# Zhengjun-Du/LC-CRF-SLAM

Measured on AMD Instinct MI355X. Metric: CRF mean-field iters/sec, higher is better.
Workload: dtype f32; 1 GPU; C2: 2000 keypoints, 5 iters, two 2-D kernels (TUM3.yaml), L=2; frames_in_flight_per_gpu=16384, handles=1, distinct_frames=64, n_points=2000, n_iters=5, n_labels=2, engine=fused

## Files before the change

### lc-crf-slam_amd/csrc/fused_lean.h

```cpp
#pragma once

#include "fused_loop.h"

#ifndef LCCRF_LEAN_SKIP
#define LCCRF_LEAN_SKIP 0
#endif
#define LEAN_SKIP(bit) ((LCCRF_LEAN_SKIP & (bit)) != 0)

namespace lccrf {
namespace fl {

constexpr int kLeanMaxRounds = 4;
__host__ __device__ constexpr int lean_rounds(int nt) { return nt >= 512 ? 3 : 4; }
__host__ __device__ constexpr int lean_max_v(int nt) { return 3 * (nt - 64); }

__host__ __device__ inline int lean_plane_floats(int NA, int V0)
{
    const int top = V0 < kChainTop ? V0 : kChainTop;
    return (NA * kD1 + 11 * top + 3 * (V0 - top) + 16 + 63) & ~63;
}

__host__ __device__ inline bool lean_chain_wanted(int NA, int V0, int row0, int nt)
{
    return row0 >= kChainMinRow && V0 <= chain_max_v(nt) && V0 <= 256 && lean_plane_floats(NA, V0) < 65535;
}

struct LeanTables {
    int val0, val1, nbr, row;
};
__host__ __device__ inline LeanTables lean_tables(size_t &o, int Vk, bool chain)
{
    auto take = [&](size_t bytes) { size_t r = o; o += (bytes + 15) & ~(size_t)15; return (int)r; };
    LeanTables t;
    t.val0 = take((size_t)(Vk + 1) * sizeof(float2));
    t.val1 = take((size_t)(Vk + 1) * sizeof(float2));
    t.nbr = chain ? take((size_t)kD1 * Vk * sizeof(unsigned)) : -1;
    t.row = take((size_t)(Vk + 2) * sizeof(unsigned short));
    return t;
}

__host__ __device__ inline bool layout_lean(int NA, int K, const int *V, int row0, FusedLayout *lay, int nt, size_t lds_limit)
{
    constexpr int D1 = kD1;
    if (NA < 1 || K < 1 || K > kMaxFusedK) return false;
    for (int k = 0; k < K; ++k)
        if (V[k] >= 65535 || V[k] > lean_max_v(nt)) return false;
    if (row0 >= kChainMinRow && !lean_chain_wanted(NA, V[0], row0, nt)) return false;
    const int chain0 = lean_chain_wanted(NA, V[0], row0, nt);
    {
        FusedLayout L{};
        size_t o = 0;
        auto take = [&](size_t bytes) { size_t r = o; o += (bytes + 15) & ~(size_t)15; return (int)r; };
        L.prod_all = 0;
        L.chain0 = chain0;
        L.zero = take(128);
        size_t shared_prod = 0;
        for (int k = 0; k < K; ++k) {
            const bool chain = k == 0 && chain0;
            L.Ecap[k] = chain ? lean_plane_floats(NA, V[k]) : ((NA * D1 + 63) & ~63);
            const LeanTables lt = lean_tables(o, V[k], chain);
            L.val[k][0] = lt.val0;
            L.val[k][1] = lt.val1;
            L.nbr[k] = lt.nbr;
            L.row[k] = lt.row;
            const size_t pb = (size_t)L.Ecap[k] * 2 * sizeof(float);
            shared_prod = pb > shared_prod ? pb : shared_prod;
        }
        if (o > 65535) return false;
        L.pstart = chain0 ? take((size_t)(V[0] + 2) * sizeof(unsigned short)) : 0;
        const int p = take(shared_prod < 1024 ? 1024 : shared_prod);
        for (int k = 0; k < K; ++k) L.prod[k] = p;
        L.total = (int)o;
        if (o <= lds_limit) {
            *lay = L;
            return true;
        }
    }
    return false;
}

#define LCCRF_ASM_SEL(off, vlo, vhi, S)                                                                             \
    "v_cmp_lt_i32_e32 vcc, " #off ", %[rem]\n\tv_cndmask_b32_e32 %[" #S "], 0, %[ad], vcc\n\t"                     \
    "ds_read_b128 v[" #vlo ":" #vhi "], %[" #S "] offset:" #off "\n\t"

__device__ __forceinline__ float chain_rows_sel(unsigned addr, int bytes, unsigned trips, unsigned &keep0, unsigned &keep1)
{
    float acc = 0.0f;
    if (trips == 0) return acc;
    unsigned sa, sb;
    asm volatile(
        LCCRF_ASM_SEL(0, 96, 99, sa) LCCRF_ASM_SEL(16, 100, 103, sb)
        LCCRF_ASM_SEL(32, 104, 107, sa) LCCRF_ASM_SEL(48, 108, 111, sb)
        LCCRF_ASM_SEL(64, 112, 115, sa) LCCRF_ASM_SEL(80, 116, 119, sb)
        "1:\n\t"
        LCCRF_ASM_SEL(96, 120, 123, sa) LCCRF_ASM_SEL(112, 124, 127, sb)
        "s_waitcnt lgkmcnt(6)\n\t"
        LCCRF_ASM_ADD8(v96, v97, v98, v99, v100, v101, v102, v103)
        "v_add_u32_e32 %[ad], 0x80, %[ad]\n\t"
        "v_subrev_u32_e32 %[rem], 0x80, %[rem]\n\t"
        LCCRF_ASM_SEL(0, 96, 99, sa) LCCRF_ASM_SEL(16, 100, 103, sb)
        "s_waitcnt lgkmcnt(6)\n\t"
        LCCRF_ASM_ADD8(v104, v105, v106, v107, v108, v109, v110, v111)
        LCCRF_ASM_SEL(32, 104, 107, sa) LCCRF_ASM_SEL(48, 108, 111, sb)
        "s_waitcnt lgkmcnt(6)\n\t"
        LCCRF_ASM_ADD8(v112, v113, v114, v115, v116, v117, v118, v119)
        LCCRF_ASM_SEL(64, 112, 115, sa) LCCRF_ASM_SEL(80, 116, 119, sb)
        "s_waitcnt lgkmcnt(6)\n\t"
        LCCRF_ASM_ADD8(v120, v121, v122, v123, v124, v125, v126, v127)
        "s_sub_u32 %[n], %[n], 1\n\t"
        "s_cmp_lg_u32 %[n], 0\n\t"
        "s_cbranch_scc1 1b\n\t"
        "s_waitcnt lgkmcnt(0)\n\t"
        : [acc] "+v"(acc), [ad] "+v"(addr), [rem] "+v"(bytes), [n] "+s"(trips), [sa] "=&v"(sa), [sb] "=&v"(sb), "+v"(keep0), "+v"(keep1)
        :
        : "scc", "vcc", "memory", LCCRF_CHAIN_RING_CLOBBERS);
    return acc;
}

__device__ __forceinline__ float chain_rows_keep(unsigned addr, unsigned end, unsigned trips, unsigned &keep0, unsigned &keep1)
{
    float acc = 0.0f;
    if (trips == 0) return acc;
    const unsigned e1 = end - 32u, e2 = end - 64u, e3 = end - 96u;
    unsigned sel;
    asm volatile(LCCRF_CHAIN_ROWS_ASM
                 : [acc] "+v"(acc), [ad] "+v"(addr), [n] "+s"(trips), [sel] "=&v"(sel), "+v"(keep0), "+v"(keep1)
                 : [e0] "v"(end), [e1] "v"(e1), [e2] "v"(e2), [e3] "v"(e3)
                 : "scc", "memory", LCCRF_CHAIN_RING_CLOBBERS);
    return acc;
}

__device__ __forceinline__ float2 lds_f2(unsigned addr)
{
#if defined(__HIP_DEVICE_COMPILE__)
    typedef float lean_f2 __attribute__((ext_vector_type(2)));
    const lean_f2 v = *reinterpret_cast<const __attribute__((address_space(3))) lean_f2 *>((unsigned long)addr);
    return make_float2(v.x, v.y);
#else
    (void)addr;
    return make_float2(0.f, 0.f);
#endif
}

__device__ __forceinline__ void lds_store_f(unsigned addr, float v)
{
#if defined(__HIP_DEVICE_COMPILE__)
    *reinterpret_cast<__attribute__((address_space(3))) float *>((unsigned long)addr) = v;
#else
    (void)addr; (void)v;
#endif
}
__device__ __forceinline__ void lds_store_f2(unsigned addr, float a, float b)
{
#if defined(__HIP_DEVICE_COMPILE__)
    typedef float lean_f2 __attribute__((ext_vector_type(2)));
    lean_f2 v;
    v.x = a;
    v.y = b;
    *reinterpret_cast<__attribute__((address_space(3))) lean_f2 *>((unsigned long)addr) = v;
#else
    (void)addr; (void)a; (void)b;
#endif
}

template <int PPT, int K, int CH>
__device__ __forceinline__ void point_products_lean(const FusedLayout &lay, const PointRegs<PPT, K> &pr, int s, int k)
{
    const unsigned a0 = (pr.ix[s][k][1] >> 16) << 2, a1 = (pr.ix[s][k][2] & 0xffffu) << 2, a2 = (pr.ix[s][k][2] >> 16) << 2;
    if (chain_k<CH>(lay, k)) {
        const unsigned pb = (unsigned)lay.Ecap[k] * 4u;
        lds_store_f(a0, pr.bary[s][k][0] * pr.q[s].x);
        lds_store_f(a0 + pb, pr.bary[s][k][0] * pr.q[s].y);
        lds_store_f(a1, pr.bary[s][k][1] * pr.q[s].x);
        lds_store_f(a1 + pb, pr.bary[s][k][1] * pr.q[s].y);
        lds_store_f(a2, pr.bary[s][k][2] * pr.q[s].x);
        lds_store_f(a2 + pb, pr.bary[s][k][2] * pr.q[s].y);
    } else {
        lds_store_f2(a0, pr.bary[s][k][0] * pr.q[s].x, pr.bary[s][k][0] * pr.q[s].y);
        lds_store_f2(a1, pr.bary[s][k][1] * pr.q[s].x, pr.bary[s][k][1] * pr.q[s].y);
        lds_store_f2(a2, pr.bary[s][k][2] * pr.q[s].x, pr.bary[s][k][2] * pr.q[s].y);
    }
}

template <int PPT, int K>
__device__ __forceinline__ float2 slice_point_lean(const PointRegs<PPT, K> &pr, int s, int k, float alpha)
{
    const float2 x0 = lds_f2(pr.ix[s][k][0] & 0xffffu), x1 = lds_f2(pr.ix[s][k][0] >> 16), x2 = lds_f2(pr.ix[s][k][1] & 0xffffu);
    const float w0 = pr.bary[s][k][0] * alpha, w1 = pr.bary[s][k][1] * alpha, w2 = pr.bary[s][k][2] * alpha;
    float t0 = w0 * x0.x, t1 = w0 * x0.y;
    t0 += w1 * x1.x; t1 += w1 * x1.y;
    t0 += w2 * x2.x; t1 += w2 * x2.y;
    return make_float2(t0, t1);
}

template <int NT>
__device__ __forceinline__ ChainLane chain_setup_lean(unsigned char *smem, const FusedLayout &lay, int V0, int tid)
{
    constexpr int k = 0;
    ChainLane cl{0u, 0u};
    int *hist = reinterpret_cast<int *>(smem + lay.prod[k]);
    if (tid < 128) hist[tid] = 0;
    __syncthreads();
    const unsigned short *row = reinterpret_cast<const unsigned short *>(smem + lay.row[k]);
    unsigned short *srt = reinterpret_cast<unsigned short *>(smem + lay.prod[k]) + 256;
    unsigned short *pstart = reinterpret_cast<unsigned short *>(smem + lay.pstart);
    int key = 0;
    if (tid < V0) {
        const int len = (int)row[tid + 1] - (int)row[tid];
        key = 63 - min((len + 3) >> 4, 63);
        atomicAdd(&hist[key], 1);
    }
    __syncthreads();
    if (tid < 64) {
        const int x = hist[tid];
        int incl = x;
#pragma unroll
        for (int o = 1; o < 64; o <<= 1) {
            const int y = __shfl_up(incl, o, 64);
            if (tid >= o) incl += y;
        }
        hist[64 + tid] = incl - x;
    }
    __syncthreads();
    if (tid < V0) srt[atomicAdd(&hist[64 + key], 1)] = (unsigned short)tid;
    __syncthreads();
    if (tid < 64) {
        int sz[4], sum = 0;
#pragma unroll
        for (int u = 0; u < 4; ++u) {
            const int r = tid * 4 + u;
            sz[u] = 0;
            if (r < V0) {
                const int v = srt[r];
                const int rl = (int)row[v + 1] - (int)row[v];
                sz[u] = ((rl + 3) & ~3) + (r < kChainTop ? 8 : 0);
            }
            sum += sz[u];
        }
        int incl = sum;
#pragma unroll
        for (int o = 1; o < 64; o <<= 1) {
            const int y = __shfl_up(incl, o, 64);
            if (tid >= o) incl += y;
        }
        int base = incl - sum;
#pragma unroll
        for (int u = 0; u < 4; ++u) {
            const int r = tid * 4 + u;
            if (r < V0) pstart[srt[r]] = (unsigned short)base;
            base += sz[u];
        }
    }
    __syncthreads();
    const int l = (tid >> 6) & 1, pr = tid >> 7, ln = tid & 63;
    const int r = pr == 0 ? (chain_top_rank(ln) >= 0 ? chain_top_rank(ln) : V0) : kChainTop + ((pr - 1) << 6) + ln;
    unsigned quads = 0, addr = 0;
    if (r < V0) {
        const int v = srt[r];
        const int rl = (int)row[v + 1] - (int)row[v], len4 = (rl + 3) & ~3;
        addr = (unsigned)(lay.prod[k] + 4 * (l * lay.Ecap[k] + (int)pstart[v]));
        quads = (unsigned)(len4 >> 2);
        cl.b = quads | ((unsigned)(len4 - rl) << 13) | ((unsigned)((v + 1) * 2 + l) << 16);
    }
    unsigned m = quads;
#pragma unroll
    for (int o = 32; o > 0; o >>= 1) m = max(m, (unsigned)__shfl_xor((int)m, o));
    cl.a = addr | (m << 18);
    __syncthreads();
    return cl;
}

__device__ __forceinline__ void chain_pads_lean(unsigned char *smem, const ChainLane &cl, int tid)
{
    if (cl.b >> 16) {
        float *e = reinterpret_cast<float *>(smem + (cl.a & 0x3ffffu)) + (cl.b & 0x1fffu) * 4u;
        const unsigned npad = (cl.b >> 13) & 3u;
        for (unsigned z = 1; z <= npad; ++z) e[-(int)z] = 0.0f;
        if ((tid >> 7) == 0) {
            reinterpret_cast<float4 *>(e)[0] = make_float4(0.f, 0.f, 0.f, 0.f);
            reinterpret_cast<float4 *>(e)[1] = make_float4(0.f, 0.f, 0.f, 0.f);
        }
    }
}

template <int PPT, int K, int CH, int NT>
__device__ __forceinline__ void place_products_lean(unsigned char *smem, const FusedLayout &lay, int N, int tid,
                                                    const unsigned (&pk)[PPT][K][kD1], PointRegs<PPT, K> &pr)
{
#pragma unroll
    for (int k = 0; k < K; ++k) {
        const unsigned short *row = reinterpret_cast<const unsigned short *>(smem + lay.row[k]);
        const unsigned short *pstart = reinterpret_cast<const unsigned short *>(smem + lay.pstart);
#pragma unroll
        for (int s = 0; s < PPT; ++s) {
            const unsigned vb = (unsigned)lay.val[k][kD1 & 1];
            pr.ix[s][k][0] = (vb + 8u * (pk[s][k][0] & 0xffffu)) | ((vb + 8u * (pk[s][k][1] & 0xffffu)) << 16);
            pr.ix[s][k][1] = vb + 8u * (pk[s][k][2] & 0xffffu);
            pr.ix[s][k][2] = 0;
            if (tid + s * NT < N) {
                unsigned sl[kD1];
#pragma unroll
                for (int j = 0; j < kD1; ++j) {
                    sl[j] = pk[s][k][j] >> 16;
                    if (chain_k<CH>(lay, k)) {
                        const int v = (int)(pk[s][k][j] & 0xffffu) - 1;
                        sl[j] = (unsigned)((int)pstart[v] + ((int)(pk[s][k][j] >> 16) - (int)row[v]));
                        sl[j] = ((unsigned)lay.prod[k] >> 2) + sl[j];
                    } else {
                        sl[j] = ((unsigned)lay.prod[k] >> 2) + 2u * sl[j];
                    }
                }
                pr.ix[s][k][1] |= sl[0] << 16;
                pr.ix[s][k][2] = sl[1] | (sl[2] << 16);
            }
        }
    }
}

typedef unsigned lean_u3 __attribute__((ext_vector_type(3)));
struct LeanSrc {
    __amdgpu_buffer_rsrc_t nbr[kMaxFusedK];
    __amdgpu_buffer_rsrc_t bary[kMaxFusedK];
    __amdgpu_buffer_rsrc_t norm[kMaxFusedK];
    __amdgpu_buffer_rsrc_t unary;
    int nbr_axis_bytes[kMaxFusedK];
    int off_nbr[kMaxFusedK], off_bary[kMaxFusedK], off_norm[kMaxFusedK], off_unary;
};
constexpr int kLeanRecPoints = 4 * kNTSmall;
constexpr int kLeanRecUnary = 0;
constexpr int kLeanRecBary = kLeanRecUnary + kLeanRecPoints * 8;
constexpr int kLeanRecNorm = kLeanRecBary + kMaxFusedK * kLeanRecPoints * kD1 * 4;
constexpr int kLeanRecNbr = kLeanRecNorm + kMaxFusedK * kLeanRecPoints * 4;
constexpr int kLeanRecNbrAxis = lean_max_v(kNTSmall) * 4;
constexpr int kLeanRecBytes = (kLeanRecNbr + kD1 * kLeanRecNbrAxis + 255) & ~255;
__device__ __forceinline__ __amdgpu_buffer_rsrc_t lean_rsrc(const void *p, size_t bytes)
{
    return __builtin_amdgcn_make_buffer_rsrc(const_cast<void *>(p), 0, (int)bytes, 0x00020000);
}

template <int PPT, int K>
__device__ __forceinline__ void opaque_ids(PointRegs<PPT, K> &pr)
{
#pragma unroll
    for (int s = 0; s < PPT; ++s) {
#pragma unroll
        for (int k = 0; k < K; ++k) asm volatile("" : "+v"(pr.ix[s][k][0]), "+v"(pr.ix[s][k][1]), "+v"(pr.ix[s][k][2]));
    }
}

struct LeanPrepPlan {
    int cl_off;
    int row_off[kMaxFusedK], row_bytes[kMaxFusedK];
    int nbr_off[kMaxFusedK], nbr_bytes[kMaxFusedK];
    int total;
};
__host__ __device__ inline LeanPrepPlan lean_prep_plan(const FusedLayout &lay, int K, const int *Vcap, int nt, int ppt)
{
    LeanPrepPlan p{};
    int o = K * ppt * nt * 12;
    p.cl_off = o;
    o += nt * 8;
    for (int k = 0; k < K; ++k) {
        p.row_off[k] = o;
        p.row_bytes[k] = ((Vcap[k] + 2) * 2 + 15) & ~15;
        o += p.row_bytes[k];
        p.nbr_off[k] = o;
        p.nbr_bytes[k] = lay.nbr[k] >= 0 ? ((kD1 * Vcap[k] * 4 + 15) & ~15) : 0;
        o += p.nbr_bytes[k];
    }
    p.total = (o + 255) & ~255;
    return p;
}

template <int PPT, int K, int CH, int NT, bool RELOAD, bool NORM = false, bool PRELOADED = false>
__device__ __forceinline__ void mean_field_lean(unsigned char *smem, const FusedLayout &lay, const int (&V)[K], int N, int &t,
                                                PointRegs<PPT, K> &pr, ChainLane &cl, const float (&alpha)[K],
                                                const float (&wk)[K], const LeanSrc &src, int n_iter, float relax, float omr, Instr &ins)
{
    constexpr int D1 = kD1;
    constexpr int KF = K - 1;
    const int wave_base = __builtin_amdgcn_readfirstlane(t & ~63);
    (void)wave_base;
#define LEAN_FRESH_T()                                                                                               \
    do {                                                                                                             \
        int z_ = 0;                                                                                                  \
        asm volatile("" : "+v"(z_));                                                                                 \
        t = wave_base + (int)__builtin_amdgcn_mbcnt_hi(~0u, __builtin_amdgcn_mbcnt_lo(~0u, (unsigned)z_));          \
    } while (0)
    auto load_weights = [&]() {
        if (!RELOAD) return;
#pragma unroll
        for (int s = 0; s < PPT; ++s) {
            const int i = t + s * NT;
            if (!NORM) {
                typedef unsigned lean_u2 __attribute__((ext_vector_type(2)));
                const lean_u2 u = __builtin_amdgcn_raw_buffer_load_b64(src.unary, i * 8, src.off_unary, 0);
                pr.un[s] = make_float2(__uint_as_float(u.x), __uint_as_float(u.y));
            }
#pragma unroll
            for (int k = 0; k < K; ++k) {
                const lean_u3 b = __builtin_amdgcn_raw_buffer_load_b96(src.bary[k], i * (D1 * 4), src.off_bary[k], 0);
                pr.bary[s][k][0] = __uint_as_float(b.x);
                pr.bary[s][k][1] = __uint_as_float(b.y);
                pr.bary[s][k][2] = __uint_as_float(b.z);
                if (!NORM) pr.wn[s][k] = __uint_as_float(__builtin_amdgcn_raw_buffer_load_b32(src.norm[k], i * 4, src.off_norm[k], 0));
            }
        }
        if (NORM) return;
#pragma unroll
        for (int s = 0; s < PPT; ++s)
#pragma unroll
            for (int k = 0; k < K; ++k) pr.wn[s][k] = wk[k] * pr.wn[s][k];
    };
    auto phase_P = [&](int k) {
#pragma unroll
        for (int s = 0; s < PPT; ++s)
            if (t + s * NT < N) point_products_lean<PPT, K, CH>(lay, pr, s, k);
        if (chain_k<CH>(lay, k)) chain_pads_lean(smem, cl, t);
    };
    auto phase_S = [&](int k) {
        float *val = reinterpret_cast<float *>(smem + lay.val[k][0]);
        if (chain_k<CH>(lay, k)) {
            const int npairs = 1 + ((max(V[k] - kChainTop, 0) + 63) >> 6);
            if (__builtin_expect((t >> 7) < npairs, 1)) {
                FL_PSTAMP();
                if ((t >> 7) == 0) __builtin_amdgcn_s_setprio(3);
                asm volatile("" : "+v"(cl.a), "+v"(cl.b));
                if (__builtin_expect((cl.b >> 16) != 0, 1) && !LEAN_SKIP(2)) {
                    const unsigned row_addr = cl.a & 0x3ffffu, row_end = row_addr + (cl.b & 0x1fffu) * 16u;
                    const unsigned m = (unsigned)__builtin_amdgcn_readfirstlane((int)(cl.a >> 18));
                    const float acc = (t >> 7) == 0 ? chain_rows_keep(row_addr, row_end, (((m + 1u) >> 1) + 3u) >> 2, cl.a, cl.b)
                                                      : chain_rows_sel(row_addr, (int)((cl.b & 0x1fffu) * 16u), (m + 7u) >> 3, cl.a, cl.b);
                    val[cl.b >> 16] = acc;
                }
                LEAN_FRESH_T();
                if ((t >> 7) == 0) __builtin_amdgcn_s_setprio(0);
                FL_PSTAMP();
            }
            return;
        }
        if (LEAN_SKIP(32)) return;
        const float2 *pl = reinterpret_cast<const float2 *>(smem + lay.prod[k]);
        const float2 *zero = reinterpret_cast<const float2 *>(smem + lay.zero);
        const unsigned short *row = reinterpret_cast<const unsigned short *>(smem + lay.row[k]);
        constexpr int RS = (K == 2 && CH == 0) ? 1 : lean_rounds(NT);
        for (int base = 0; base < lean_rounds(NT); base += RS) {
            int p0[RS], pe[RS];
#pragma unroll
            for (int r = 0; r < RS; ++r) {
                const int v = t + (base + r) * NT;
                p0[r] = pe[r] = 0;
                if (v < V[k]) { p0[r] = row[v]; pe[r] = row[v + 1]; }
            }
            float2 x[RS][8];
#pragma unroll
            for (int r = 0; r < RS; ++r) {
                const unsigned base = (unsigned)lay.prod[k] + 8u * (unsigned)p0[r];
                const int n = pe[r] - p0[r];
#pragma unroll
                for (int u = 0; u < 8; ++u) x[r][u] = lds_f2(((u < n) ? base : 0u) + 8u * u);
            }
#pragma unroll
            for (int r = 0; r < RS; ++r) {
                const int v = t + (base + r) * NT;
                float a0 = 0.0f, a1 = 0.0f;
#pragma unroll
                for (int u = 0; u < 8; ++u) { a0 += x[r][u].x; a1 += x[r][u].y; }
                for (int p = p0[r] + 8; p < pe[r] && !LEAN_SKIP(16); p += 8) {
                    float2 y[8];
#pragma unroll
                    for (int u = 0; u < 8; ++u) y[u] = *((p + u < pe[r]) ? pl + p + u : zero);
#pragma unroll
                    for (int u = 0; u < 8; ++u) { a0 += y[u].x; a1 += y[u].y; }
                }
                if (v < V[k]) reinterpret_cast<float2 *>(val)[v + 1] = make_float2(a0, a1);
            }
        }
        (void)V;
    };
    constexpr int R = lean_rounds(NT);
    constexpr int OVL_K = (K == 2 && CH == 1) ? 1 : K;
    auto load_nbr = [&](unsigned (&w)[OVL_K][D1][R]) {
#pragma unroll
        for (int k = 0; k < K; ++k) {
#pragma unroll
            for (int j = 0; j < D1; ++j) {
#pragma unroll
                for (int r = 0; r < R; ++r) {
                    w[k][j][r] = 0;
                    if (!(CH == 1 && k == 0) && (r == 0 || r * NT < V[k]))
                        w[k][j][r] = __builtin_amdgcn_raw_buffer_load_b32(src.nbr[k], (t + r * NT) * 4, src.off_nbr[k] + j * src.nbr_axis_bytes[k], 0);
                }
            }
        }
    };
    auto blur_pass = [&](int j, const unsigned (&w)[OVL_K][D1][R]) {
#pragma unroll
        for (int k = 0; k < K; ++k) {
            const float2 *src_v = reinterpret_cast<const float2 *>(smem + lay.val[k][j & 1]);
            float2 *dst = reinterpret_cast<float2 *>(smem + lay.val[k][(j & 1) ^ 1]);
            const bool in_lds = CH == 1 && k == 0;
            const unsigned *lds = reinterpret_cast<const unsigned *>(smem + (in_lds ? lay.nbr[k] : 0)) + j * V[k];
#pragma unroll
            for (int r = 0; r < (in_lds ? 1 : R); ++r) {
                const int v = t + r * NT;
                if (v < V[k]) {
                    const unsigned n = in_lds ? lds[v] : w[k][j][r];
                    const float2 o = src_v[v + 1], x = src_v[n & 0xffffu], y = src_v[n >> 16];
                    float2 u;
                    u.x = o.x + 0.5f * (x.x + y.x);
                    u.y = o.y + 0.5f * (x.y + y.y);
                    dst[v + 1] = u;
                }
            }
        }
    };
    constexpr bool OVL = K == 2 && CH == 1;
    constexpr int NA0 = NT - 128, RA = 4;
    constexpr int NB = NT - 64, RB = 3;
    auto load_nbr_ovl = [&](unsigned (&wa)[RA], unsigned (&wb)[2][RB]) {
#pragma unroll
        for (int r = 0; r < RA; ++r) {
            wa[r] = 0;
            if ((r == 0 || r * NA0 < V[K - 1]) && !LEAN_SKIP(512))
                wa[r] = __builtin_amdgcn_raw_buffer_load_b32(src.nbr[K - 1], (t - 128 + r * NA0) * 4, src.off_nbr[K - 1], 0);
        }
#pragma unroll
        for (int j = 1; j < D1; ++j) {
#pragma unroll
            for (int r = 0; r < RB; ++r) {
                wb[j - 1][r] = 0;
                if ((r == 0 || r * NB < V[K - 1]) && !LEAN_SKIP(512))
                    wb[j - 1][r] = __builtin_amdgcn_raw_buffer_load_b32(src.nbr[K - 1], (t + r * NB) * 4, src.off_nbr[K - 1] + j * src.nbr_axis_bytes[K - 1], 0);
            }
        }
    };
    auto blur_vertex = [&](const float2 *src_v, float2 *dst, int v, unsigned n) {
        if (LEAN_SKIP(64)) return;
        const float2 o = src_v[v + 1], x = src_v[n & 0xffffu], y = src_v[n >> 16];
        float2 u;
        u.x = o.x + 0.5f * (x.x + y.x);
        u.y = o.y + 0.5f * (x.y + y.y);
        dst[v + 1] = u;
    };
    auto blur_big = [&](int j, int lane, int stride, int rounds, const unsigned *w) {
        constexpr int k = K - 1;
        const float2 *src_v = reinterpret_cast<const float2 *>(smem + lay.val[k][j & 1]);
        float2 *dst = reinterpret_cast<float2 *>(smem + lay.val[k][(j & 1) ^ 1]);
#pragma unroll
        for (int r = 0; r < RA; ++r) {
            if (r < rounds) {
                const int v = lane + r * stride;
                if (v < V[k]) blur_vertex(src_v, dst, v, w[r]);
            }
        }
    };
    auto blur_small = [&](int lane, int j_lo, int j_hi) {
        const unsigned *tbl = reinterpret_cast<const unsigned *>(smem + lay.nbr[0]);
#pragma unroll
        for (int j = 0; j < D1; ++j) {
            if (j < j_lo || j >= j_hi) continue;
            const float2 *src_v = reinterpret_cast<const float2 *>(smem + lay.val[0][j & 1]);
            float2 *dst = reinterpret_cast<float2 *>(smem + lay.val[0][(j & 1) ^ 1]);
            for (int v = lane; v < V[0]; v += 64) blur_vertex(src_v, dst, v, tbl[j * V[0] + v]);
            asm volatile("s_waitcnt lgkmcnt(0)" ::: "memory");
            __builtin_amdgcn_wave_barrier();
        }
    };
    auto point_update = [&](int s) {
        if constexpr (NORM) {
#pragma unroll
            for (int k = 0; k < K; ++k) {
                const float v = slice_point_lean(pr, s, k, alpha[k]).x;
                const float nrm = 1.0f / (v + 1e-20f);
                if (RELOAD) __builtin_amdgcn_raw_buffer_store_b32(__float_as_uint(nrm), src.norm[k], (t + s * NT) * 4, src.off_norm[k], 0);
                else pr.wn[s][k] = wk[k] * nrm;
            }
            return;
        }
        float nx[2] = {-pr.un[s].x, -pr.un[s].y};
#pragma unroll
        for (int k = 0; k < K; ++k) {
            const float2 t = slice_point_lean(pr, s, k, alpha[k]);
            nx[0] += pr.wn[s][k] * t.x;
            nx[1] += pr.wn[s][k] * t.y;
        }
        pr.q[s] = softmax2(nx[0], nx[1], pr.q[s], relax, omr);
    };

    if (n_iter <= 0) return;
    if (!PRELOADED) load_weights();
#pragma unroll
    for (int s = 0; s < PPT; ++s)
        if (t + s * NT < N) point_products_lean<PPT, K, CH>(lay, pr, s, KF);
    if (chain_k<CH>(lay, KF)) chain_pads_lean(smem, cl, t);
    for (int it = 0; it < n_iter; ++it) {
        LEAN_FRESH_T();
        if (RELOAD) opaque_ids(pr);
        else opaque(pr);
        unsigned w[OVL ? 1 : K][D1][R];
        unsigned wa[RA], wb[2][RB];
        if constexpr (OVL) load_nbr_ovl(wa, wb);
        else load_nbr(w);
        __syncthreads();
        FL_STAMP();
        phase_S(KF);
#pragma unroll
        for (int k = KF - 1; k >= 0; --k) {
            __syncthreads();
            opaque_ids(pr);
            phase_P(k);
            __syncthreads();
            phase_S(k);
        }
        if constexpr (OVL) {
            if (t >= 128) blur_big(0, t - 128, NA0, RA, wa);
            __syncthreads();
            FL_STAMP();
            LEAN_FRESH_T();
            if (t >= NB) blur_small(t - NB, 0, 2);
            else blur_big(1, t, NB, RB, wb[0]);
            __syncthreads();
            if (!NORM && !LEAN_SKIP(256)) load_weights();
            if (t < NB) blur_big(2, t, NB, RB, wb[1]);
            else blur_small(t - NB, 2, D1);
            __syncthreads();
        } else {
            __syncthreads();
            FL_STAMP();
            LEAN_FRESH_T();
            blur_pass(0, w);
            __syncthreads();
            blur_pass(1, w);
            __syncthreads();
            if (!NORM && !LEAN_SKIP(256)) load_weights();
            blur_pass(2, w);
            __syncthreads();
        }
        FL_STAMP();
        LEAN_FRESH_T();
        opaque_ids(pr);
        const bool more = it + 1 < n_iter;
#pragma unroll
        for (int s = 0; s < PPT; ++s) {
            if (t + s * NT < N && !LEAN_SKIP(128)) {
                point_update(s);
                if (more) point_products_lean<PPT, K, CH>(lay, pr, s, KF);
            }
        }
        FL_STAMP();
    }
}

#undef LEAN_FRESH_T

}
}
```

### lc-crf-slam_amd/csrc/fused_loop.h

```cpp
#pragma once

#include "engine.h"
#include "device_math.h"

namespace lccrf {
namespace fl {

constexpr int kNT = 1024;
constexpr int kMaxFusedK = 2;
constexpr int kD1 = 3;
constexpr int kChainGap = 14;
constexpr int kChainTop = 16;
__host__ __device__ constexpr int chain_top_rank(int ln)
{
    return ((ln & 0x18) == 0) ? ((ln & 7) | ((ln >> 5) << 3)) : -1;
}
constexpr size_t kLdsLimit = 160 * 1024;
constexpr int kChainMinRow = 64;
__host__ __device__ constexpr int chain_max_v(int nt) { return kChainTop + (nt / 128 - 1) * 64; }
constexpr int kChainMaxV = chain_max_v(kNT);
constexpr int kNTSmall = 512;
constexpr int kSmallMinFrames = 256;
constexpr size_t kLdsHalf = kLdsLimit / 2;

#ifndef LCCRF_INSTRUMENT
#define LCCRF_INSTRUMENT 0
#endif
constexpr bool kInstr = LCCRF_INSTRUMENT != 0;

struct FusedLayout {
    int zero;
    int prod[kMaxFusedK];
    int val[kMaxFusedK][2];
    int nbr[kMaxFusedK];
    int row[kMaxFusedK];
    int Ecap[kMaxFusedK];
    int prod_all;
    int chain0;
    int pstart;
    int total;
};

struct Instr {
    long long *timing;
    int timing_block;
    int dbg;
    int n;
    int lane;
};
#define FL_DBG(bit) (::lccrf::fl::kInstr && (ins.dbg & (bit)))
#define FL_STAMP()                                                                                                   \
    do {                                                                                                             \
        if (::lccrf::fl::kInstr && ins.timing && (int)blockIdx.x == ins.timing_block && (int)threadIdx.x == ins.lane) ins.timing[ins.n++] = clock64(); \
    } while (0)
#define FL_PSTAMP()                   \
    do {                              \
        if (FL_DBG(8)) FL_STAMP();    \
    } while (0)

__host__ __device__ inline int pst(int r0, int v) { return (r0 + kChainGap * v + 3) & ~3; }

__host__ __device__ inline int plane_floats(int NA, int V, bool chain) { return ((chain ? NA * kD1 + kChainGap * V + 16 : NA * kD1) + 63) & ~63; }

__host__ __device__ inline bool chain_wanted(int NA, int V0, int row0, int nt = kNT)
{
    return row0 >= kChainMinRow && V0 <= chain_max_v(nt) && NA * kD1 + kChainGap * V0 + 64 < 65535;
}

__host__ __device__ inline bool layout_core(int NA, int K, const int *V, int row0, FusedLayout *lay, int nt = kNT,
                                            size_t lds_limit = kLdsLimit)
{
    constexpr int D1 = kD1;
    if (NA < 1 || NA > 4 * kNT || K < 1 || K > kMaxFusedK) return false;
    for (int k = 0; k < K; ++k)
        if (V[k] >= 65535) return false;
    const int chain0 = chain_wanted(NA, V[0], row0, nt);
    for (int all = 1; all >= 0; --all) {
        FusedLayout L{};
        size_t o = 0;
        auto take = [&](size_t bytes) { size_t r = o; o += (bytes + 15) & ~(size_t)15; return (int)r; };
        L.prod_all = all;
        L.chain0 = chain0;
        (void)take(128);
        L.zero = take(64);
        size_t shared_prod = 0;
        for (int k = 0; k < K; ++k) {
            L.Ecap[k] = plane_floats(NA, V[k], k == 0 && chain0);
            L.val[k][0] = take((size_t)(V[k] + 1) * sizeof(float2));
            L.val[k][1] = take((size_t)(V[k] + 1) * sizeof(float2));
            L.nbr[k] = take((size_t)D1 * V[k] * sizeof(unsigned));
            L.row[k] = take((size_t)(V[k] + 2) * sizeof(unsigned short));
            const size_t pb = (size_t)L.Ecap[k] * 2 * sizeof(float);
            if (all) L.prod[k] = take(pb);
            else shared_prod = pb > shared_prod ? pb : shared_prod;
        }
        if (!all) {
            const int p = take(shared_prod);
            for (int k = 0; k < K; ++k) L.prod[k] = p;
        }
        L.total = (int)o;
        if (o <= lds_limit) {
            *lay = L;
            return true;
        }
    }
    return false;
}

#define LCCRF_ASM_ADD8(a, b, c, d, e, f, g, h)                                                        \
    "v_add_f32_e32 %[acc], %[acc], " #a "\n\tv_add_f32_e32 %[acc], %[acc], " #b "\n\t"               \
    "v_add_f32_e32 %[acc], %[acc], " #c "\n\tv_add_f32_e32 %[acc], %[acc], " #d "\n\t"               \
    "v_add_f32_e32 %[acc], %[acc], " #e "\n\tv_add_f32_e32 %[acc], %[acc], " #f "\n\t"               \
    "v_add_f32_e32 %[acc], %[acc], " #g "\n\tv_add_f32_e32 %[acc], %[acc], " #h "\n\t"

#define LCCRF_CHAIN_ROWS_ASM                                                                                         \
        "v_min_u32_e32 %[sel], %[ad], %[e0]\n\t"                                                                     \
        "ds_read_b128 v[96:99], %[sel]\n\tds_read_b128 v[100:103], %[sel] offset:16\n\t"                             \
        "v_min_u32_e32 %[sel], %[ad], %[e1]\n\t"                                                                     \
        "ds_read_b128 v[104:107], %[sel] offset:32\n\tds_read_b128 v[108:111], %[sel] offset:48\n\t"                 \
        "v_min_u32_e32 %[sel], %[ad], %[e2]\n\t"                                                                     \
        "ds_read_b128 v[112:115], %[sel] offset:64\n\tds_read_b128 v[116:119], %[sel] offset:80\n\t"                 \
        "1:\n\t"                                                                                                     \
        "v_min_u32_e32 %[sel], %[ad], %[e3]\n\t"                                                                     \
        "ds_read_b128 v[120:123], %[sel] offset:96\n\tds_read_b128 v[124:127], %[sel] offset:112\n\t"                \
        "s_waitcnt lgkmcnt(6)\n\t"                                                                                   \
        LCCRF_ASM_ADD8(v96, v97, v98, v99, v100, v101, v102, v103)                                                   \
        "v_add_u32_e32 %[ad], 0x80, %[ad]\n\t"                                                                       \
        "v_min_u32_e32 %[sel], %[ad], %[e0]\n\t"                                                                     \
        "ds_read_b128 v[96:99], %[sel]\n\tds_read_b128 v[100:103], %[sel] offset:16\n\t"                             \
        "s_waitcnt lgkmcnt(6)\n\t"                                                                                   \
        LCCRF_ASM_ADD8(v104, v105, v106, v107, v108, v109, v110, v111)                                               \
        "v_min_u32_e32 %[sel], %[ad], %[e1]\n\t"                                                                     \
        "ds_read_b128 v[104:107], %[sel] offset:32\n\tds_read_b128 v[108:111], %[sel] offset:48\n\t"                 \
        "s_waitcnt lgkmcnt(6)\n\t"                                                                                   \
        LCCRF_ASM_ADD8(v112, v113, v114, v115, v116, v117, v118, v119)                                               \
        "v_min_u32_e32 %[sel], %[ad], %[e2]\n\t"                                                                     \
        "ds_read_b128 v[112:115], %[sel] offset:64\n\tds_read_b128 v[116:119], %[sel] offset:80\n\t"                 \
        "s_waitcnt lgkmcnt(6)\n\t"                                                                                   \
        LCCRF_ASM_ADD8(v120, v121, v122, v123, v124, v125, v126, v127)                                               \
        "s_sub_u32 %[n], %[n], 1\n\t"                                                                                \
        "s_cmp_lg_u32 %[n], 0\n\t"                                                                                   \
        "s_cbranch_scc1 1b\n\t"                                                                                      \
        "s_waitcnt lgkmcnt(0)\n\t"
#define LCCRF_CHAIN_RING_CLOBBERS                                                                                      \
    "v96", "v97", "v98", "v99", "v100", "v101", "v102", "v103", "v104", "v105", "v106", "v107", "v108", "v109", "v110", "v111", "v112",   \
        "v113", "v114", "v115", "v116", "v117", "v118", "v119", "v120", "v121", "v122", "v123", "v124", "v125", "v126", "v127"

__device__ __forceinline__ float chain_rows(unsigned addr, unsigned end, unsigned trips)
{
    float acc = 0.0f;
    if (trips == 0) return acc;
    const unsigned e1 = end - 32u, e2 = end - 64u, e3 = end - 96u;
    unsigned sel;
    asm volatile(LCCRF_CHAIN_ROWS_ASM
                 : [acc] "+v"(acc), [ad] "+v"(addr), [n] "+s"(trips), [sel] "=&v"(sel)
                 : [e0] "v"(end), [e1] "v"(e1), [e2] "v"(e2), [e3] "v"(e3)
                 : "scc", "memory", LCCRF_CHAIN_RING_CLOBBERS);
    return acc;
}

template <int PPT, int K>
struct PointRegs {
    float2 un[PPT], q[PPT];
    unsigned ix[PPT][K][3];
    float bary[PPT][K][kD1];
    float wn[PPT][K];
};

struct ChainLane {
    unsigned a, b;
};

template <int CH>
__device__ __forceinline__ bool chain_k(const FusedLayout &lay, int k)
{
    return CH == 2 ? (k == 0 && lay.chain0 != 0) : (((CH >> k) & 1) != 0);
}

template <int PPT, int K, int CH, int NT = kNT, int KMASK = (1 << K) - 1>
__device__ __forceinline__ void place_products(unsigned char *smem, const FusedLayout &lay, int N, int tid,
                                               const unsigned (&pk)[PPT][K][kD1], PointRegs<PPT, K> &pr)
{
#pragma unroll
    for (int k = 0; k < K; ++k) {
        if (!((KMASK >> k) & 1)) continue;
        const unsigned short *row = reinterpret_cast<const unsigned short *>(smem + lay.row[k]);
#pragma unroll
        for (int s = 0; s < PPT; ++s) {
            pr.ix[s][k][0] = (pk[s][k][0] & 0xffffu) | (pk[s][k][1] << 16);
            pr.ix[s][k][1] = pk[s][k][2] & 0xffffu;
            pr.ix[s][k][2] = 0;
            if (tid + s * NT < N) {
                unsigned sl[kD1];
#pragma unroll
                for (int j = 0; j < kD1; ++j) {
                    sl[j] = pk[s][k][j] >> 16;
                    if (chain_k<CH>(lay, k)) {
                        const int v = (int)(pk[s][k][j] & 0xffffu) - 1;
                        const int r0 = row[v];
                        sl[j] = (unsigned)(pst(r0, v) + ((int)(pk[s][k][j] >> 16) - r0));
                    }
                }
                pr.ix[s][k][1] |= sl[0] << 16;
                pr.ix[s][k][2] = sl[1] | (sl[2] << 16);
            }
        }
    }
}

__device__ __forceinline__ ChainLane chain_setup(unsigned char *smem, const FusedLayout &lay, int V0, int tid)
{
    constexpr int k = 0;
    ChainLane cl{0u, 0u};
    int *hist = reinterpret_cast<int *>(smem + lay.prod[k]);
    if (tid < 128) hist[tid] = 0;
    __syncthreads();
    const unsigned short *row = reinterpret_cast<const unsigned short *>(smem + lay.row[k]);
    unsigned short *srt = reinterpret_cast<unsigned short *>(smem + lay.prod[k]) + 256;
    int key = 0, len = 0;
    if (tid < V0) {
        len = (int)row[tid + 1] - (int)row[tid];
        key = 63 - min((len + 3) >> 4, 63);
        atomicAdd(&hist[key], 1);
    }
    __syncthreads();
    if (tid < 64) {
        const int x = hist[tid];
        int incl = x;
#pragma unroll
        for (int o = 1; o < 64; o <<= 1) {
            const int y = __shfl_up(incl, o, 64);
            if (tid >= o) incl += y;
        }
        hist[64 + tid] = incl - x;
    }
    __syncthreads();
    if (tid < V0) srt[atomicAdd(&hist[64 + key], 1)] = (unsigned short)tid;
    __syncthreads();
    const int l = (tid >> 6) & 1, pr = tid >> 7, ln = tid & 63;
    const int r = pr == 0 ? (chain_top_rank(ln) >= 0 ? chain_top_rank(ln) : V0) : kChainTop + ((pr - 1) << 6) + ln;
    unsigned nblk = 0, addr = 0;
    if (r < V0) {
        const int v = srt[r];
        const int r0 = row[v], rl = (int)row[v + 1] - r0, len4 = (rl + 3) & ~3;
        addr = (unsigned)(lay.prod[k] + 4 * (l * lay.Ecap[k] + pst(r0, v)));
        nblk = (unsigned)((len4 + 7) >> 3);
        cl.b = nblk | ((unsigned)((len4 >> 2) & 1) << 13) | ((unsigned)(len4 - rl) << 14) | ((unsigned)((v + 1) * 2 + l) << 16);
    }
    unsigned m = nblk;
#pragma unroll
    for (int o = 32; o > 0; o >>= 1) m = max(m, (unsigned)__shfl_xor((int)m, o));
    cl.a = addr | (m << 18);
    __syncthreads();
    return cl;
}

template <int PPT, int K, int CH>
__device__ __forceinline__ void point_products(unsigned char *smem, const FusedLayout &lay, const PointRegs<PPT, K> &pr, int s, int k)
{
    float *p0 = reinterpret_cast<float *>(smem + lay.prod[k]);
    float *p1 = p0 + lay.Ecap[k];
    float2 *p2 = reinterpret_cast<float2 *>(p0);
    const unsigned s0 = pr.ix[s][k][1] >> 16, s1 = pr.ix[s][k][2] & 0xffffu, s2 = pr.ix[s][k][2] >> 16;
    if (chain_k<CH>(lay, k)) {
        p0[s0] = pr.bary[s][k][0] * pr.q[s].x;
        p1[s0] = pr.bary[s][k][0] * pr.q[s].y;
        p0[s1] = pr.bary[s][k][1] * pr.q[s].x;
        p1[s1] = pr.bary[s][k][1] * pr.q[s].y;
        p0[s2] = pr.bary[s][k][2] * pr.q[s].x;
        p1[s2] = pr.bary[s][k][2] * pr.q[s].y;
    } else {
        p2[s0] = make_float2(pr.bary[s][k][0] * pr.q[s].x, pr.bary[s][k][0] * pr.q[s].y);
        p2[s1] = make_float2(pr.bary[s][k][1] * pr.q[s].x, pr.bary[s][k][1] * pr.q[s].y);
        p2[s2] = make_float2(pr.bary[s][k][2] * pr.q[s].x, pr.bary[s][k][2] * pr.q[s].y);
    }
}

__device__ __forceinline__ void chain_pads(unsigned char *smem, const ChainLane &cl)
{
    if (cl.b >> 16) {
        float *e = reinterpret_cast<float *>(smem + (cl.a & 0x3ffffu)) + ((cl.b & 0x1fffu) * 8u - ((cl.b >> 13) & 1u) * 4u);
        const unsigned npad = (cl.b >> 14) & 3u;
        for (unsigned z = 1; z <= npad; ++z) e[-(int)z] = 0.0f;
        reinterpret_cast<float4 *>(e)[0] = make_float4(0.f, 0.f, 0.f, 0.f);
        reinterpret_cast<float4 *>(e)[1] = make_float4(0.f, 0.f, 0.f, 0.f);
    }
}

template <int PPT, int K, int CH, bool WITH_P = true, int NT = kNT, int KMASK = (1 << K) - 1, bool REV = false>
__device__ __forceinline__ void splat_blur(unsigned char *smem, const FusedLayout &lay, const int (&V)[K], int N, int tid,
                                           const PointRegs<PPT, K> &pr, const ChainLane &cl, Instr &ins)
{
    constexpr int D1 = kD1;
    auto phase_P = [&](int k) {
#pragma unroll
        for (int s = 0; s < PPT; ++s)
            if (tid + s * NT < N) point_products<PPT, K, CH>(smem, lay, pr, s, k);
        if (chain_k<CH>(lay, k)) chain_pads(smem, cl);
    };
    auto phase_S = [&](int k, int s_lo) {
        float *val = reinterpret_cast<float *>(smem + lay.val[k][0]);
        if (chain_k<CH>(lay, k)) {
            const int npairs = 1 + ((max(V[k] - kChainTop, 0) + 63) >> 6);
            if ((tid >> 7) < npairs && !FL_DBG(2)) {
                FL_PSTAMP();
                __builtin_amdgcn_s_setprio(3);
                if ((cl.b >> 16) != 0) {
                    const unsigned row_addr = cl.a & 0x3ffffu;
                    const float acc = chain_rows(row_addr, row_addr + ((cl.b & 0x1fffu) * 8u - ((cl.b >> 13) & 1u) * 4u) * 4u,
                                                 ((unsigned)__builtin_amdgcn_readfirstlane((int)(cl.a >> 18)) + 3u) >> 2);
                    val[cl.b >> 16] = acc;
                }
                __builtin_amdgcn_s_setprio(0);
                FL_PSTAMP();
            }
            return;
        }
        const float2 *pl = reinterpret_cast<const float2 *>(smem + lay.prod[k]);
        const float2 *zero = reinterpret_cast<const float2 *>(smem + lay.zero);
        const unsigned short *row = reinterpret_cast<const unsigned short *>(smem + lay.row[k]);
        if (tid < s_lo || FL_DBG(1)) return;
        for (int v = tid - s_lo; v < V[k]; v += NT - s_lo) {
            const int t = row[v + 1];
            float a0 = 0.0f, a1 = 0.0f;
            for (int p = row[v]; p < t; p += 8) {
                float2 x[8];
#pragma unroll
                for (int u = 0; u < 8; ++u) x[u] = *((p + u < t) ? pl + p + u : zero);
#pragma unroll
                for (int u = 0; u < 8; ++u) { a0 += x[u].x; a1 += x[u].y; }
            }
            reinterpret_cast<float2 *>(val)[v + 1] = make_float2(a0, a1);
        }
    };
    constexpr auto on = [](int k) { return ((KMASK >> k) & 1) != 0; };
    if (lay.prod_all) {
        if (WITH_P) {
#pragma unroll
            for (int k = 0; k < K; ++k)
                if (on(k)) phase_P(k);
        }
        __syncthreads();
        FL_STAMP();
        const int s_lo = (K > 1 && on(0) && on(1) && chain_k<CH>(lay, 0)) ? 128 : 0;
#pragma unroll
        for (int k = 0; k < K; ++k)
            if (on(k)) phase_S(k, s_lo);
        __syncthreads();
        FL_STAMP();
    } else {
#pragma unroll
        for (int k = 0; k < K; ++k) {
            if (!on(k)) continue;
            phase_P(k);
            __syncthreads();
            phase_S(k, 0);
            __syncthreads();
        }
    }

#pragma unroll
    for (int j = 0; j < D1; ++j) {
#pragma unroll
        for (int k = 0; k < K; ++k) {
            if (!on(k)) continue;
            const float2 *src = reinterpret_cast<const float2 *>(smem + lay.val[k][j & 1]);
            float2 *dst = reinterpret_cast<float2 *>(smem + lay.val[k][(j & 1) ^ 1]);
            const unsigned *nbr = reinterpret_cast<const unsigned *>(smem + lay.nbr[k]) + j * V[k];
            int v0 = tid;
            if (REV && K > 1 && k == 0 && NT == kNT) {
                asm volatile("" : "+v"(v0));
                v0 = NT - 1 - v0;
            }
            for (int v = v0; v < V[k]; v += NT) {
                const unsigned n = nbr[v];
                const float2 o = src[v + 1], x = src[n & 0xffffu], y = src[n >> 16];
                float2 r;
                r.x = o.x + 0.5f * (x.x + y.x);
                r.y = o.y + 0.5f * (x.y + y.y);
                dst[v + 1] = r;
            }
        }
        __syncthreads();
    }
    FL_STAMP();
}

template <int PPT, int K>
__device__ __forceinline__ float2 slice_point(const unsigned char *smem, const FusedLayout &lay, const PointRegs<PPT, K> &pr,
                                              int s, int k, float alpha)
{
    const float2 *val = reinterpret_cast<const float2 *>(smem + lay.val[k][kD1 & 1]);
    const float2 x0 = val[pr.ix[s][k][0] & 0xffffu], x1 = val[pr.ix[s][k][0] >> 16], x2 = val[pr.ix[s][k][1] & 0xffffu];
    const float w0 = pr.bary[s][k][0] * alpha, w1 = pr.bary[s][k][1] * alpha, w2 = pr.bary[s][k][2] * alpha;
    float t0 = w0 * x0.x, t1 = w0 * x0.y;
    t0 += w1 * x1.x; t1 += w1 * x1.y;
    t0 += w2 * x2.x; t1 += w2 * x2.y;
    return make_float2(t0, t1);
}

template <int PPT, int K>
__device__ __forceinline__ void opaque(PointRegs<PPT, K> &pr)
{
#pragma unroll
    for (int s = 0; s < PPT; ++s) {
#pragma unroll
        for (int k = 0; k < K; ++k) {
            asm volatile("" : "+v"(pr.ix[s][k][0]), "+v"(pr.ix[s][k][1]), "+v"(pr.ix[s][k][2]));
            asm volatile("" : "+v"(pr.bary[s][k][0]), "+v"(pr.bary[s][k][1]), "+v"(pr.bary[s][k][2]));
        }
    }
}

template <int PPT, int K, int NT = kNT>
__device__ __forceinline__ void start_inference(PointRegs<PPT, K> &pr, int N, int tid)
{
#pragma unroll
    for (int s = 0; s < PPT; ++s) {
        pr.q[s] = make_float2(0.f, 0.f);
        if (tid + s * NT < N) {
            pr.q[s] = softmax2(-pr.un[s].x, -pr.un[s].y, make_float2(0.f, 0.f), 1.0f);
        }
    }
}

template <int PPT, int K, int CH, int NT = kNT, bool REV = false>
__device__ __forceinline__ void mean_field(unsigned char *smem, const FusedLayout &lay, const int (&V)[K], int N, int tid,
                                           PointRegs<PPT, K> &pr, const ChainLane &cl, const float (&alpha)[K], int n_iter,
                                           float relax, Instr &ins, int first_p = -1)
{
    auto point_update = [&](int s) {
        float nx[2] = {-pr.un[s].x, -pr.un[s].y};
#pragma unroll
        for (int k = 0; k < K; ++k) {
            const float2 t = slice_point(smem, lay, pr, s, k, alpha[k]);
            nx[0] += pr.wn[s][k] * t.x;
            nx[1] += pr.wn[s][k] * t.y;
        }
        pr.q[s] = softmax2(nx[0], nx[1], pr.q[s], relax);
    };
    if (PPT <= 2 && lay.prod_all) {
        if (n_iter > 0) {
#pragma unroll
            for (int k = 0; k < K; ++k) {
                if (!((first_p >> k) & 1)) continue;
#pragma unroll
                for (int s = 0; s < PPT; ++s)
                    if (tid + s * NT < N) point_products<PPT, K, CH>(smem, lay, pr, s, k);
                if (chain_k<CH>(lay, k)) chain_pads(smem, cl);
            }
        }
        for (int it = 0; it < n_iter; ++it) {
            opaque(pr);
            splat_blur<PPT, K, CH, false, NT, (1 << K) - 1, REV>(smem, lay, V, N, tid, pr, cl, ins);
            const bool more = it + 1 < n_iter;
#pragma unroll
            for (int s = 0; s < PPT; ++s) {
                if (tid + s * NT < N) {
                    point_update(s);
                    if (more) {
#pragma unroll
                        for (int k = 0; k < K; ++k) point_products<PPT, K, CH>(smem, lay, pr, s, k);
                    }
                }
            }
            FL_STAMP();
        }
        return;
    }
    for (int it = 0; it < n_iter; ++it) {
        opaque(pr);
        splat_blur<PPT, K, CH, true, NT, (1 << K) - 1, REV>(smem, lay, V, N, tid, pr, cl, ins);
#pragma unroll
        for (int s = 0; s < PPT; ++s)
            if (tid + s * NT < N) point_update(s);
        FL_STAMP();
    }
}

template <int NT>
__device__ __forceinline__ void clear_label_bits(const CrfDev &c, int f, int first_word, int tid)
{
    if (c.map_bits)
        for (int w = first_word + tid; w < c.bits_stride; w += NT) c.map_bits[(size_t)f * c.bits_stride + w] = 0ull;
}

template <int PPT, int K, int NT = kNT>
__device__ __forceinline__ void store_results(const CrfDev &c, int f, int N, int tid, const PointRegs<PPT, K> &pr, int with_map)
{
#pragma unroll
    for (int s = 0; s < PPT; ++s) {
        const int i = tid + s * NT;
        if (i < N) {
            reinterpret_cast<float2 *>(c.Q)[(size_t)f * c.maxN + i] = pr.q[s];
            if (with_map) c.map[(size_t)f * c.maxN + i] = (pr.q[s].x < pr.q[s].y) ? 1 : 0;
        }
        if (with_map && c.map_bits && (i & ~63) < N) {
            const unsigned long long m = __ballot(i < N && pr.q[s].x < pr.q[s].y);
            if ((tid & 63) == 0) c.map_bits[(size_t)f * c.bits_stride + (i >> 6)] = m;
        }
    }
    if (with_map) clear_label_bits<NT>(c, f, (N + 63) >> 6, tid);
}

}
}
```

Baseline: 48.29 million iters/s.

## Pack both labels of the chain top rows into one wavefront

The top chain rows for both labels are now handled by a single 64-lane wavefront instead of two. A new lane map assigns label and rank per lane so that each ds_read_b128 lane group holds one label. This frees the second wavefront, which now joins the first blur pass (NA0 = NT-64, RA = 3) instead of idling. Compile-time checks confirm the lane map. The risk is a heavier critical-path wave in the chain phase, plus possible LDS bank conflicts.

After: 48.60 million iters/s, median of 6. Within noise of the previous version (+0.7%).

```diff
diff --git a/lc-crf-slam_amd/csrc/fused_lean.h b/lc-crf-slam_amd/csrc/fused_lean.h
--- a/lc-crf-slam_amd/csrc/fused_lean.h
+++ b/lc-crf-slam_amd/csrc/fused_lean.h
@@ -252,8 +252,9 @@
         }
     }
     __syncthreads();
-    const int l = (tid >> 6) & 1, pr = tid >> 7, ln = tid & 63;
-    const int r = pr == 0 ? (chain_top_rank(ln) >= 0 ? chain_top_rank(ln) : V0) : kChainTop + ((pr - 1) << 6) + ln;
+    const int pr = tid >> 7, ln = tid & 63;
+    const int l = pr == 0 ? chain_top_lane_label(ln) : (tid >> 6) & 1;
+    const int r = pr == 0 ? (((tid >> 6) == 0 && chain_top_lane_rank(ln) >= 0) ? chain_top_lane_rank(ln) : V0) : kChainTop + ((pr - 1) << 6) + ln;
     unsigned quads = 0, addr = 0;
     if (r < V0) {
         const int v = srt[r];
@@ -276,7 +277,7 @@
         float *e = reinterpret_cast<float *>(smem + (cl.a & 0x3ffffu)) + (cl.b & 0x1fffu) * 4u;
         const unsigned npad = (cl.b >> 13) & 3u;
         for (unsigned z = 1; z <= npad; ++z) e[-(int)z] = 0.0f;
-        if ((tid >> 7) == 0) {
+        if ((tid >> 6) == 0) {
             reinterpret_cast<float4 *>(e)[0] = make_float4(0.f, 0.f, 0.f, 0.f);
             reinterpret_cast<float4 *>(e)[1] = make_float4(0.f, 0.f, 0.f, 0.f);
         }
@@ -422,19 +423,19 @@
         float *val = reinterpret_cast<float *>(smem + lay.val[k][0]);
         if (chain_k<CH>(lay, k)) {
             const int npairs = 1 + ((max(V[k] - kChainTop, 0) + 63) >> 6);
-            if (__builtin_expect((t >> 7) < npairs, 1)) {
+            if (__builtin_expect((t >> 7) < npairs && (t >> 6) != 1, 1)) {
                 FL_PSTAMP();
-                if ((t >> 7) == 0) __builtin_amdgcn_s_setprio(3);
+                if ((t >> 6) == 0) __builtin_amdgcn_s_setprio(3);
                 asm volatile("" : "+v"(cl.a), "+v"(cl.b));
                 if (__builtin_expect((cl.b >> 16) != 0, 1) && !LEAN_SKIP(2)) {
                     const unsigned row_addr = cl.a & 0x3ffffu, row_end = row_addr + (cl.b & 0x1fffu) * 16u;
                     const unsigned m = (unsigned)__builtin_amdgcn_readfirstlane((int)(cl.a >> 18));
-                    const float acc = (t >> 7) == 0 ? chain_rows_keep(row_addr, row_end, (((m + 1u) >> 1) + 3u) >> 2, cl.a, cl.b)
+                    const float acc = (t >> 6) == 0 ? chain_rows_keep(row_addr, row_end, (((m + 1u) >> 1) + 3u) >> 2, cl.a, cl.b)
                                                       : chain_rows_sel(row_addr, (int)((cl.b & 0x1fffu) * 16u), (m + 7u) >> 3, cl.a, cl.b);
                     val[cl.b >> 16] = acc;
                 }
                 LEAN_FRESH_T();
-                if ((t >> 7) == 0) __builtin_amdgcn_s_setprio(0);
+                if ((t >> 6) == 0) __builtin_amdgcn_s_setprio(0);
                 FL_PSTAMP();
             }
             return;
@@ -516,14 +517,14 @@
         }
     };
     constexpr bool OVL = K == 2 && CH == 1;
-    constexpr int NA0 = NT - 128, RA = 4;
+    constexpr int NA0 = NT - 64, RA = 3;
     constexpr int NB = NT - 64, RB = 3;
     auto load_nbr_ovl = [&](unsigned (&wa)[RA], unsigned (&wb)[2][RB]) {
 #pragma unroll
         for (int r = 0; r < RA; ++r) {
             wa[r] = 0;
             if ((r == 0 || r * NA0 < V[K - 1]) && !LEAN_SKIP(512))
-                wa[r] = __builtin_amdgcn_raw_buffer_load_b32(src.nbr[K - 1], (t - 128 + r * NA0) * 4, src.off_nbr[K - 1], 0);
+                wa[r] = __builtin_amdgcn_raw_buffer_load_b32(src.nbr[K - 1], (t - 64 + r * NA0) * 4, src.off_nbr[K - 1], 0);
         }
 #pragma unroll
         for (int j = 1; j < D1; ++j) {
@@ -614,7 +615,7 @@
             phase_S(k);
         }
         if constexpr (OVL) {
-            if (t >= 128) blur_big(0, t - 128, NA0, RA, wa);
+            if (t >= 64) blur_big(0, t - 64, NA0, RA, wa);
             __syncthreads();
             FL_STAMP();
             LEAN_FRESH_T();
diff --git a/lc-crf-slam_amd/csrc/fused_loop.h b/lc-crf-slam_amd/csrc/fused_loop.h
--- a/lc-crf-slam_amd/csrc/fused_loop.h
+++ b/lc-crf-slam_amd/csrc/fused_loop.h
@@ -10,11 +10,42 @@
 constexpr int kMaxFusedK = 2;
 constexpr int kD1 = 3;
 constexpr int kChainGap = 14;
-constexpr int kChainTop = 16;
+#ifndef LCCRF_CHAIN_TOP
+#define LCCRF_CHAIN_TOP 16
+#endif
+constexpr int kChainTop = LCCRF_CHAIN_TOP;
+static_assert(kChainTop == 8 || kChainTop == 16, "the lean loop's lane map (chain_top_lane_rank) is written for 8 or 16 rows");
 __host__ __device__ constexpr int chain_top_rank(int ln)
 {
-    return ((ln & 0x18) == 0) ? ((ln & 7) | ((ln >> 5) << 3)) : -1;
-}
+    return ((ln & (32 - kChainTop / 2) & 31) == 0) ? ((ln & (kChainTop / 2 - 1)) | ((ln >> 5) << (kChainTop == 16 ? 3 : 2))) : -1;
+}
+__host__ __device__ constexpr int chain_top_lane_label(int ln)
+{
+    return kChainTop == 8 ? ((ln >> 2) & 1) : ((((ln & 15) + 4) >> 3) & 1);
+}
+__host__ __device__ constexpr int chain_top_lane_rank(int ln)
+{
+    return kChainTop == 8 ? (((ln & 0x18) == 0) ? ((ln & 3) + (ln >> 5) * 4) : -1)
+                          : (((ln & 0x10) == 0) ? (((ln + 4) & 7) + (ln >> 5) * 8) : -1);
+}
+constexpr int ds128_group(int ln) { return (ln >> 5) * 2 + ((((ln & 31) >= 4 && (ln & 31) < 12) || ((ln & 31) >= 16 && (ln & 31) < 20) || (ln & 31) >= 28) ? 1 : 0); }
+constexpr bool chain_top_lane_map_ok()
+{
+    int seen[2][kChainTop] = {}, per_group[4] = {};
+    for (int ln = 0; ln < 64; ++ln) {
+        const int r = chain_top_lane_rank(ln), l = chain_top_lane_label(ln);
+        if (r < 0) continue;
+        if (r >= kChainTop || l != (ds128_group(ln) & 1)) return false;
+        ++seen[l][r];
+        ++per_group[ds128_group(ln)];
+    }
+    for (int r = 0; r < kChainTop; ++r)
+        if (seen[0][r] != 1 || seen[1][r] != 1) return false;
+    for (int g = 0; g < 4; ++g)
+        if (per_group[g] != kChainTop / 2) return false;
+    return true;
+}
+static_assert(chain_top_lane_map_ok(), "chain_top_lane_rank / chain_top_lane_label");
 constexpr size_t kLdsLimit = 160 * 1024;
 constexpr int kChainMinRow = 64;
 __host__ __device__ constexpr int chain_max_v(int nt) { return kChainTop + (nt / 128 - 1) * 64; }
```
